# dataexplorations2026/cough_detector

Hardware: AMD Instinct MI355X
Metric: 1s@16kHz clips/sec (featurise+infer) (higher is better)
Workload: dtype bf16x3: split-bf16 MFMA (feature image, activations and BN-folded weights as hi+lo bf16 pairs, 3 v_mfma_f32_32x32x16_bf16 per k-step, f32 accumulate, f32 activations in HBM); featuriser f32

## Files before the change

cough_detector_amd/csrc/featurize.hip:

```cpp
#include <cmath>
#include <cstddef>
#include <cstring>
#include <type_traits>
#include <vector>

#include <hip/hip_bf16.h>

#include <cstdlib>

#include "common.h"
#include "fft256.h"
#include "internal.h"

namespace cough {
namespace {

constexpr int NS = 16000, NFFT = 512, HOP = 160, WIN = 400, NFRAMES = 101, NMEL = 64, NMFCC = 13;
constexpr int PADL = NFFT / 2;
constexpr int NBIN = 128;
constexpr int MAXW = 8;
constexpr int THREADS = 256, WAVES = THREADS / 64;
constexpr int FPW = 4;
constexpr int NGROUP = (NFRAMES + FPW - 1) / FPW;
constexpr int XROW = 17;
constexpr int XFRAME = 16 * XROW;
constexpr int NMF = NMFCC * NFRAMES;
constexpr int FIRST_PLAIN = 2, LAST_PLAIN = 98;

struct FeatTables {
    float win[NFFT];
    float2 tw256[16][16];
    float2 tw512[NBIN];
    int mel_start[NMEL];
    float mel_w[NMEL][MAXW];
    float dct_t[NMFCC + 1][NMEL];
};

constexpr size_t LDS_XCH = size_t(WAVES) * FPW * XFRAME * 4;
constexpr size_t LDS_MEL = size_t(NMEL) * NFRAMES * 4;
constexpr size_t LDS_RED = 16 * 4;
constexpr size_t LDS_TW = size_t(16) * XROW * 8;
constexpr size_t LDS_TOTAL = LDS_XCH + LDS_MEL + LDS_RED + LDS_TW;
static_assert(LDS_TOTAL * 3 <= 160 * 1024, "three workgroups per CU");
static_assert(LDS_XCH >= size_t(2) * NMF * 4, "MFCC / delta buffers alias the transpose scratch");

__device__ __forceinline__ float block_max(float v, float* red, int tid) {
    v = wave_max(v);
    __syncthreads();
    if ((tid & 63) == 0) red[tid >> 6] = v;
    __syncthreads();
    float r = red[0];
#pragma unroll
    for (int w = 1; w < WAVES; ++w) r = fmaxf(r, red[w]);
    return r;
}
__device__ __forceinline__ float block_sum(float v, float* red, int tid) {
    v = wave_sum(v);
    __syncthreads();
    if ((tid & 63) == 0) red[tid >> 6] = v;
    __syncthreads();
    float r = red[0];
#pragma unroll
    for (int w = 1; w < WAVES; ++w) r += red[w];
    return r;
}

#ifdef COUGH_K1_STAMPS
__device__ unsigned long long* g_stamp_buf = nullptr;
#define K1_STAMP(slot)                                                                      \
    do {                                                                                    \
        if (g_stamp_buf && threadIdx.x == 0)                                                \
            g_stamp_buf[(size_t)blockIdx.x * 8 + (slot)] = __builtin_amdgcn_s_memtime();    \
    } while (0)
#else
#define K1_STAMP(slot) do { } while (0)
#endif

#ifdef COUGH_K1_MARKERS
#define K1_MARK(text)                             \
    do {                                          \
        __builtin_amdgcn_sched_barrier(0);        \
        asm volatile("; K1MARK " text);           \
        __builtin_amdgcn_sched_barrier(0);        \
    } while (0)
#else
#define K1_MARK(text) do { } while (0)
#endif

using f32x16 = __attribute__((ext_vector_type(16))) float;
using bf16x8 = __attribute__((ext_vector_type(8))) __bf16;
__device__ __forceinline__ uint16_t f2bf(float f) {
    __hip_bfloat16 b = __float2bfloat16(f);
    return *reinterpret_cast<uint16_t*>(&b);
}
constexpr int ST_P1H = 22, ST_P1W = 25, ST_ROWS = 94, ST_PITCH = 106;
constexpr int ST_PER = ST_P1H * ST_P1W, ST_TILES = (ST_PER + 7) / 8;
constexpr size_t ST_IMG = size_t(ST_ROWS) * ST_PITCH * 2;
static_assert(ST_IMG <= LDS_MEL, "the bf16 feature image aliases the dB buffer");
constexpr size_t ST_X3_OFF = LDS_TOTAL - 2 * ST_IMG;
static_assert(ST_X3_OFF % 16 == 0 && ST_IMG % 4 == 0 && ST_X3_OFF >= size_t(NMF) * 4, "hi / lo images vs the MFCC buffer");

struct FullBank {
    int n_mels, n_mfcc, n_taps;
    int maxw[2];
    int n_frames, n_samples, hop;
    int cph, cph_pad, cw;
    const int *lo, *hi, *off;
    const float* w;
    const float* dct;
};
constexpr size_t full_mel_bytes(int n_mels, int n_frames = NFRAMES) { return (size_t(n_mels) * n_frames * 4 + 15) & ~size_t(15); }
constexpr int FX_ROW = FPW * 16 + 1, FX_WAVE = 16 * FX_ROW, FX_PROW = 260;
static_assert(FPW * FX_PROW <= FX_WAVE && FX_PROW >= NFFT / 2 + 2 && FX_PROW % 2 == 0, "four power rows replace the transposes");
constexpr size_t LDS_XCH_FULL = size_t(WAVES) * FX_WAVE * 4;
constexpr int FULL_MAX_MFCC = int(LDS_XCH_FULL / (size_t(2) * NFRAMES * 4));
constexpr size_t full_lds_bytes(int n_mels, int n_taps, int n_frames = NFRAMES) {
    return LDS_XCH_FULL + full_mel_bytes(n_mels, n_frames) + LDS_RED + LDS_TW + ((size_t(n_taps) * 4 + 15) & ~size_t(15));
}

#ifndef COUGH_GEO_WG_PER_CU
#define COUGH_GEO_WG_PER_CU 2
#endif
template <bool PRE_EMPH, int STEM, bool FULL = false, bool TALL = false, bool PCS = false, bool GEO = false>
__global__ __launch_bounds__(THREADS, GEO ? COUGH_GEO_WG_PER_CU : 3) void featurize_kernel(
    const float* __restrict__ wav, long long wav_stride, float* __restrict__ out, int nfeat,
    const FeatTables* __restrict__ tb, int normalize, float pre_coef, int delta_delta , int pcen, StemFuse stem, FullBank fbk,
    const float* __restrict__ full_dct ,
    float* __restrict__ peak_out ) {
    extern __shared__ __attribute__((aligned(16))) char smem[];
    static_assert(!GEO || (FULL && STEM == 0 && !TALL && !PCS), "run-time geometry: full-band instantiations without a stem");
    const int NF = GEO ? fbk.n_frames : NFRAMES, NGR = GEO ? (fbk.n_frames + FPW - 1) / FPW : NGROUP;
    const int NSMP = GEO ? fbk.n_samples : NS, HP = GEO ? fbk.hop : HOP;
    constexpr int N1A = GEO ? 0 : 1, N1B = GEO ? 16 : 15;
    const int nmel = FULL ? fbk.n_mels : NMEL, nmfcc = FULL ? fbk.n_mfcc : NMFCC, nmf = nmfcc * NF;
    const size_t lds_mel = FULL ? full_mel_bytes(nmel, NF) : LDS_MEL;
    constexpr size_t lds_xch = FULL ? LDS_XCH_FULL : LDS_XCH;
    float* xs = reinterpret_cast<float*>(smem);
    float* melbuf = reinterpret_cast<float*>(smem + lds_xch);
    float* red = reinterpret_cast<float*>(smem + lds_xch + lds_mel);
    float2* twl = reinterpret_cast<float2*>(smem + lds_xch + lds_mel + LDS_RED);
    float* c_w = reinterpret_cast<float*>(smem + lds_xch + lds_mel + LDS_RED + LDS_TW);

    const int tid = threadIdx.x, lane = tid & 63, wave = tid >> 6;
    const long long clip = blockIdx.x;
    const float* x = wav + clip * wav_stride;
    float* o = out + clip * (long long)nfeat * NF;
    const bool wr = out != nullptr;

    K1_STAMP(0);
    K1_STAMP(1);
    K1_MARK("PHASE prologue (window taps, twiddle table, mel taps to registers)");

    const int j = lane & 15, fsub = lane >> 4;
    twl[(tid >> 4) * XROW + (tid & 15)] = tb->tw256[tid >> 4][tid & 15];
    int b_lo[2] = {0, 0}, b_w[2] = {0, 0}, b_band[2] = {0, 0};
    const float* b_taps[2] = {c_w, c_w};
    int fpl1 = FPW;
    if constexpr (FULL) {
        for (int i = tid; i < fbk.n_taps; i += THREADS) c_w[i] = fbk.w[i];
        const int r = nmel - 64;
        fpl1 = r > 32 ? 4 : r > 16 ? 2 : 1;
#pragma unroll
        for (int ps = 0; ps < 2; ++ps) {
            const int mb = ps == 0 ? lane : 64 + (fpl1 == 4 ? lane : fpl1 == 2 ? (lane & 31) : (lane & 15));
            if (mb < nmel) {
                b_band[ps] = mb;
                b_lo[ps] = fbk.lo[mb];
                b_w[ps] = fbk.hi[mb] - b_lo[ps];
                b_taps[ps] = c_w + fbk.off[mb];
            } else {
                b_band[ps] = -1;
            }
        }
    }
    __syncthreads();
    const float2* tw_row = twl + j * XROW;
    const float2 tw_j = tb->tw512[j];
    float mw[MAXW];
#pragma unroll
    for (int q = 0; q < MAXW; ++q) mw[q] = tb->mel_w[lane][q];
    const int mstart = tb->mel_start[lane];

    float* myx = xs + (wave * FPW + fsub) * XFRAME;
    float* myw = xs + wave * FX_WAVE;
    float* fxw = myw + 16 * fsub + j;
    const float* fxr = myw + FX_ROW * j + 16 * fsub;
    float* prow = myw + FX_PROW * fsub;
    float run_max = -INFINITY;
    float peak = 0.f;
    float chk = 0.f;
    auto geo_plain = [&](int g) {
        return HP * (FPW * g) - PADL >= 0 && FPW * g + FPW - 1 < NF && HP * (FPW * g + FPW - 1) - PADL + NFFT <= NSMP;
    };
    [[maybe_unused]] float raw_left = 0.f;
    auto load_group = [&](int g, float2 (&raw)[16]) {
        const int t_raw = FPW * g + fsub;
        const int t = t_raw < NF ? t_raw : NF - 1;
        const int s0 = HP * t - PADL + 2 * j;
        if constexpr (GEO) {
            if (geo_plain(g)) {
#pragma unroll
                for (int n1 = 0; n1 < 16; ++n1) raw[n1] = make_float2(x[s0 + 32 * n1], x[s0 + 32 * n1 + 1]);
                if constexpr (PRE_EMPH) raw_left = s0 - 2 * j > 0 ? x[s0 - 2 * j - 1] : 0.f;
            } else {
#pragma unroll
                for (int n1 = 0; n1 < 16; ++n1) {
                    int i0 = s0 + 32 * n1, i1 = i0 + 1;
                    i0 = i0 < 0 ? -i0 : (i0 >= NSMP ? 2 * (NSMP - 1) - i0 : i0);
                    i1 = i1 < 0 ? -i1 : (i1 >= NSMP ? 2 * (NSMP - 1) - i1 : i1);
                    raw[n1] = make_float2(x[i0], x[i1]);
                }
            }
        } else
        if (FPW * g >= FIRST_PLAIN && FPW * g + FPW - 1 <= LAST_PLAIN) {
            K1_MARK("WEIGHT 0.885 (23 of 26 groups: frames inside the clip)");
#pragma unroll
            for (int n1 = 1; n1 < 15; ++n1) raw[n1] = *reinterpret_cast<const float2*>(x + s0 + 32 * n1);
            K1_MARK("ENDWEIGHT");
        } else {
            K1_MARK("WEIGHT 0.115 (3 of 26 groups: reflected edge frames)");
#pragma unroll
            for (int n1 = 1; n1 < 15; ++n1) {
                int i0 = s0 + 32 * n1, i1 = i0 + 1;
                i0 = i0 < 0 ? -i0 : (i0 >= NS ? 2 * (NS - 1) - i0 : i0);
                i1 = i1 < 0 ? -i1 : (i1 >= NS ? 2 * (NS - 1) - i1 : i1);
                raw[n1] = make_float2(x[i0], x[i1]);
            }
            K1_MARK("ENDWEIGHT");
        }
    };
    float2 raw[16];
    float peak_m = 0.f;
    auto p1_pass = [&](const float ws1, const float ws2) {
        float w_re[16], w_im[16];
        const int jw = 2 * j;
#pragma unroll
        for (int n1 = N1A; n1 < N1B; ++n1) {
            w_re[n1] = tb->win[32 * n1 + jw] * ws1 * ws2;
            w_im[n1] = tb->win[32 * n1 + jw + 1] * ws1 * ws2;
        }
        load_group(wave, raw);

        K1_MARK("LOOP 6.5 P1 four-frame groups per wave");
        for (int g = wave; g < NGR; g += WAVES) {
            K1_MARK("PHASE P1 peak + window multiply + next group's loads");
            const int t_raw = FPW * g + fsub;
// ... 399 lines not shown
    if constexpr (TALL) {
        static_assert(!TALL || STEM == 2, "the 103-row stem: split-bf16 operands");
        constexpr int TL_P1H = 26, TL_HALF = 13, TL_PER = TL_HALF * ST_P1W, TL_ROWS = 58, TL_PLANE = TL_ROWS * ST_PITCH;
        constexpr size_t TL_IMG_OFF = (size_t(2) * NMF * 4 + 15) & ~size_t(15), TL_STASH_OFF = TL_IMG_OFF + size_t(2) * TL_PLANE * 2;
        constexpr int TL_KEEP0 = 2 * 2 * TL_HALF - 3;
        static_assert(TL_STASH_OFF % 16 == 0 && TL_STASH_OFF + size_t(NMEL - TL_KEEP0) * NFRAMES * 4 <= LDS_TOTAL, "103-row stem LDS");
        static_assert(2 * (2 * (TL_HALF - 1) + 1) + 1 + 6 < TL_ROWS && TL_P1H == 2 * TL_HALF, "partial image rows");
        constexpr int NDV = (NMEL * NFRAMES / 2 + THREADS - 1) / THREADS;
        float2 dv[NDV];
#pragma unroll
        for (int it = 0; it < NDV; ++it) {
            const int i2 = tid + it * THREADS;
            dv[it] = i2 < NMEL * NFRAMES / 2 ? reinterpret_cast<const float2*>(melbuf)[i2] : make_float2(0.f, 0.f);
        }
        float* o_mfcc = o + NMEL * NFRAMES;
        float* o_delta = o_mfcc + NMF;
        for (int item = tid; item < NMF; item += THREADS) {
            const int c = item / NFRAMES, t = item - c * NFRAMES;
            const float* row = mf + c * NFRAMES;
            const float d = (row[t < NFRAMES - 1 ? t + 1 : t] - row[t > 0 ? t - 1 : 0]) / 2.0f;
            if (wr) {
                o_mfcc[item] = row[t];
                o_delta[item] = d;
            }
            dl[item] = d;
        }
        __syncthreads();
        auto ddelta = [&](int c, int t) {
            const float* row = dl + c * NFRAMES;
            return (row[t < NFRAMES - 1 ? t + 1 : t] - row[t > 0 ? t - 1 : 0]) / 2.0f;
        };
        if (wr) {
            float* o_dd = o_delta + NMF;
            for (int item = tid; item < NMF; item += THREADS) o_dd[item] = ddelta(item / NFRAMES, item % NFRAMES);
        }
        uint16_t* timg = reinterpret_cast<uint16_t*>(smem + TL_IMG_OFF);
        float* stash = reinterpret_cast<float*>(smem + TL_STASH_OFF);
        auto tput = [&](int idx, float v) {
            const uint16_t hi = f2bf(v);
            timg[idx] = hi;
            timg[TL_PLANE + idx] = f2bf(v - __uint_as_float(uint32_t(hi) << 16));
        };
        auto zero_image = [&]() {
            for (int i = tid; i < 2 * TL_PLANE / 8; i += THREADS) reinterpret_cast<uint4*>(timg)[i] = make_uint4(0, 0, 0, 0);
            for (int i = (2 * TL_PLANE / 8) * 8 + tid; i < 2 * TL_PLANE; i += THREADS) timg[i] = 0;
            __syncthreads();
        };
        zero_image();
        if constexpr (PCS) {
            const int m = tid >> 2, t0 = (tid & 3) * 26;
#pragma unroll
            for (int k = 0; k < 26; ++k) {
                if (t0 + k < NFRAMES) {
                    if (m + 3 < TL_ROWS - 1) tput((m + 3) * ST_PITCH + t0 + k + 3, pcv[k]);
                    if (m >= TL_KEEP0) stash[(m - TL_KEEP0) * NFRAMES + t0 + k] = pcv[k];
                }
            }
        } else {
            {
#pragma unroll
                for (int it = 0; it < NDV; ++it) {
                    const int e = 2 * (tid + it * THREADS);
                    if (e < NMEL * NFRAMES) {
                        const int m0 = e / NFRAMES, t0 = e - m0 * NFRAMES;
                        const int m1 = t0 + 1 < NFRAMES ? m0 : m0 + 1, t1 = t0 + 1 < NFRAMES ? t0 + 1 : 0;
                        const float v0 = fminf(fmaxf((dv[it].x + 80.0f) * 0.0125f, 0.f), 1.f);
                        const float v1 = fminf(fmaxf((dv[it].y + 80.0f) * 0.0125f, 0.f), 1.f);
                        if (m0 + 3 < TL_ROWS - 1) tput((m0 + 3) * ST_PITCH + t0 + 3, v0);
                        if (m1 + 3 < TL_ROWS - 1) tput((m1 + 3) * ST_PITCH + t1 + 3, v1);
                        if (m0 >= TL_KEEP0) stash[(m0 - TL_KEEP0) * NFRAMES + t0] = v0;
                        if (m1 >= TL_KEEP0) stash[(m1 - TL_KEEP0) * NFRAMES + t1] = v1;
                    }
                }
            }
        }
        const int sr = lane & 31, sh = lane >> 5;
        bf16x8 bw[2][4];
#pragma unroll
        for (int pl = 0; pl < 2; ++pl)
#pragma unroll
            for (int st = 0; st < 4; ++st)
                bw[pl][st] = *reinterpret_cast<const bf16x8*>(stem.wfrag + pl * 2048 + ((st * 2 + sh) * 32 + sr) * 8);
        const float bn = stem.bias[sr];
        const int q = sr >> 2, dy = (sr >> 1) & 1, dx = sr & 1;
        float* oa = reinterpret_cast<float*>(stem.a1) + clip * (long long)(TL_P1H * ST_P1W) * 32;
#pragma unroll 1
        for (int half = 0; half < 2; ++half) {
            if (half == 1) {
                zero_image();
                for (int i = tid; i < (NMEL - TL_KEEP0) * NFRAMES; i += THREADS) {
                    const int m = i / NFRAMES, t = i - m * NFRAMES;
                    tput(m * ST_PITCH + t + 3, stash[i]);
                }
                for (int item = tid; item < NMF; item += THREADS) {
                    const int c = item / NFRAMES, t = item - c * NFRAMES;
                    tput((NMEL - TL_KEEP0 + c) * ST_PITCH + t + 3, mf[item]);
                    tput((NMEL - TL_KEEP0 + NMFCC + c) * ST_PITCH + t + 3, dl[item]);
                    tput((NMEL - TL_KEEP0 + 2 * NMFCC + c) * ST_PITCH + t + 3, ddelta(c, t));
                }
            }
            __syncthreads();
            auto tl_base = [&](int tile) -> const uint32_t* {
                int P = tile * 8 + q;
                if (P >= TL_PER) P = TL_PER - 1;
                const int ph = P / ST_P1W, pw = P - ph * ST_P1W;
                return reinterpret_cast<const uint32_t*>(timg + (2 * (2 * ph + dy) + sh) * ST_PITCH + 2 * (2 * pw + dx));
            };
            auto tl_load = [&](const uint32_t* base, bf16x8 (&fa)[2][4]) {
#pragma unroll
                for (int pl = 0; pl < 2; ++pl)
#pragma unroll
                    for (int st = 0; st < 4; ++st) {
                        const uint32_t* pp = base + pl * (TL_PLANE / 2) + st * ST_PITCH;
                        union { uint32_t u[4]; bf16x8 v; } tv;
                        tv.u[0] = pp[0]; tv.u[1] = pp[1]; tv.u[2] = pp[2]; tv.u[3] = pp[3];
                        fa[pl][st] = tv.v;
                    }
            };
            auto tl_mma = [&](const bf16x8 (&fa)[2][4], f32x16& c) {
#pragma unroll
                for (int st = 0; st < 4; ++st) {
                    c = __builtin_amdgcn_mfma_f32_32x32x16_bf16(fa[0][st], bw[0][st], c, 0, 0, 0);
                    c = __builtin_amdgcn_mfma_f32_32x32x16_bf16(fa[1][st], bw[0][st], c, 0, 0, 0);
                    c = __builtin_amdgcn_mfma_f32_32x32x16_bf16(fa[0][st], bw[1][st], c, 0, 0, 0);
                }
            };
            auto tl_store = [&](int tile, const f32x16& acc2) {
#pragma unroll
                for (int g = 0; g < 4; ++g) {
                    const int Po = tile * 8 + 2 * g + sh;
                    float v = fmaxf(fmaxf(acc2[4 * g], acc2[4 * g + 1]), fmaxf(acc2[4 * g + 2], acc2[4 * g + 3])) + bn;
                    v = fmaxf(v, 0.f);
                    if (Po < TL_PER) oa[(half * TL_PER + Po) * 32 + sr] = v;
                }
            };
            constexpr int TL_TILES = (TL_PER + 7) / 8;
            for (int ta = wave; ta < TL_TILES; ta += 2 * WAVES) {
                const int tb = ta + WAVES;
                const bool two = tb < TL_TILES;
                bf16x8 fa[2][4], fb[2][4];
                tl_load(tl_base(ta), fa);
                tl_load(tl_base(two ? tb : ta), fb);
                f32x16 ca = {0}, cb = {0};
                tl_mma(fa, ca);
                tl_mma(fb, cb);
                tl_store(ta, ca);
                if (two) tl_store(tb, cb);
            }
            __syncthreads();
        }
        return;
    }
    if constexpr (STEM != 0) {
        float2 dv[(NMEL * NFRAMES / 2 + THREADS - 1) / THREADS];
#pragma unroll
        for (int it = 0; it < (NMEL * NFRAMES / 2 + THREADS - 1) / THREADS; ++it) {
            const int i2 = tid + it * THREADS;
            dv[it] = i2 < NMEL * NFRAMES / 2 ? reinterpret_cast<const float2*>(melbuf)[i2] : make_float2(0.f, 0.f);
        }
        __syncthreads();
        constexpr int NIMG = STEM == 2 ? 2 : 1;
        for (int i = tid; i < NIMG * ST_ROWS * ST_PITCH / 8; i += THREADS) reinterpret_cast<uint4*>(img)[i] = make_uint4(0, 0, 0, 0);
        for (int i = (NIMG * ST_ROWS * ST_PITCH / 8) * 8 + tid; i < NIMG * ST_ROWS * ST_PITCH; i += THREADS) img[i] = 0;
        __syncthreads();
        if constexpr (PCS) {
            const int m = tid >> 2, t0 = (tid & 3) * 26;
#pragma unroll
            for (int k = 0; k < 26; ++k)
                if (t0 + k < NFRAMES) put((m + 3) * ST_PITCH + t0 + k + 3, pcv[k]);
        } else {
#pragma unroll
            for (int it = 0; it < (NMEL * NFRAMES / 2 + THREADS - 1) / THREADS; ++it) {
                const int e = 2 * (tid + it * THREADS);
                if (e < NMEL * NFRAMES) {
                    const int m0 = e / NFRAMES, t0 = e - m0 * NFRAMES;
                    const int m1 = t0 + 1 < NFRAMES ? m0 : m0 + 1, t1 = t0 + 1 < NFRAMES ? t0 + 1 : 0;
                    put((m0 + 3) * ST_PITCH + t0 + 3, fminf(fmaxf((dv[it].x + 80.0f) * 0.0125f, 0.f), 1.f));
                    put((m1 + 3) * ST_PITCH + t1 + 3, fminf(fmaxf((dv[it].y + 80.0f) * 0.0125f, 0.f), 1.f));
                }
            }
        }
    }
    float* o_mfcc = o + nmel * NF;
    float* o_delta = o_mfcc + nmf;
    for (int item = tid; item < nmf; item += THREADS) {
        const int c = item / NF, t = item - c * NF;
        const float* row = mf + c * NF;
        const float d = (row[t < NF - 1 ? t + 1 : t] - row[t > 0 ? t - 1 : 0]) / 2.0f;
        if (wr) {
            o_mfcc[item] = row[t];
            o_delta[item] = d;
        }
        if (delta_delta == 1) dl[item] = d;
        if constexpr (STEM != 0) {
            put((NMEL + c + 3) * ST_PITCH + t + 3, row[t]);
            put((NMEL + NMFCC + c + 3) * ST_PITCH + t + 3, d);
        }
    }
    K1_STAMP(6);
    if (delta_delta == 1 && wr) {
        __syncthreads();
        float* o_dd = o_delta + nmf;
        for (int item = tid; item < nmf; item += THREADS) {
            const int c = item / NF, t = item - c * NF;
            const float* row = dl + c * NF;
            o_dd[item] = (row[t < NF - 1 ? t + 1 : t] - row[t > 0 ? t - 1 : 0]) / 2.0f;
        }
    }
    if constexpr (STEM != 0) {
        __syncthreads();
        K1_MARK("PHASE K2 stem MFMA + pool + store");
        constexpr int NP = STEM == 2 ? 2 : 1;
        const int sr = lane & 31, sh = lane >> 5;
        bf16x8 bw[NP][4];
#pragma unroll
        for (int pl = 0; pl < NP; ++pl)
#pragma unroll
            for (int st = 0; st < 4; ++st)
                bw[pl][st] = *reinterpret_cast<const bf16x8*>(stem.wfrag + pl * 2048 + ((st * 2 + sh) * 32 + sr) * 8);
        const float bn = stem.bias[sr];
        const int q = sr >> 2, dy = (sr >> 1) & 1, dx = sr & 1;
        using out_t = std::conditional_t<STEM == 2, float, uint16_t>;
        out_t* oa = reinterpret_cast<out_t*>(stem.a1) + clip * (long long)ST_PER * 32;
        auto frag_base = [&](int tile) -> const uint32_t* {
            int P = tile * 8 + q;
            if (P >= ST_PER) P = ST_PER - 1;
            const int ph = P / ST_P1W, pw = P - ph * ST_P1W;
            return reinterpret_cast<const uint32_t*>(img + (2 * (2 * ph + dy) + sh) * ST_PITCH + 2 * (2 * pw + dx));
        };
        auto load_frags = [&](const uint32_t* base, bf16x8 (&a)[NP][4]) {
#pragma unroll
            for (int pl = 0; pl < NP; ++pl)
#pragma unroll
                for (int st = 0; st < 4; ++st) {
                    const uint32_t* p = base + pl * (ST_ROWS * ST_PITCH / 2) + st * ST_PITCH;
                    union { uint32_t u[4]; bf16x8 v; } t;
                    t.u[0] = p[0]; t.u[1] = p[1]; t.u[2] = p[2]; t.u[3] = p[3];
                    a[pl][st] = t.v;
                }
        };
        auto mma = [&](const bf16x8 (&a)[NP][4], f32x16& c) {
#pragma unroll
            for (int st = 0; st < 4; ++st) {
                c = __builtin_amdgcn_mfma_f32_32x32x16_bf16(a[0][st], bw[0][st], c, 0, 0, 0);
                if constexpr (STEM == 2) {
                    c = __builtin_amdgcn_mfma_f32_32x32x16_bf16(a[1][st], bw[0][st], c, 0, 0, 0);
                    c = __builtin_amdgcn_mfma_f32_32x32x16_bf16(a[0][st], bw[1][st], c, 0, 0, 0);
                }
            }
        };
        auto epilogue = [&](int tile, const f32x16& acc2, bool guard) {
#pragma unroll
            for (int g = 0; g < 4; ++g) {
                const int Po = tile * 8 + 2 * g + sh;
                float v = fmaxf(fmaxf(acc2[4 * g], acc2[4 * g + 1]), fmaxf(acc2[4 * g + 2], acc2[4 * g + 3])) + bn;
                v = fmaxf(v, 0.f);
                if (!guard || Po < ST_PER) {
                    if constexpr (STEM == 2) oa[Po * 32 + sr] = v;
                    else oa[Po * 32 + sr] = f2bf(v);
                }
            }
        };
        static_assert(ST_TILES == 17 * WAVES + 1, "stem tile split");
        for (int it = 0; it < 16; it += 2) {
            const int ta = wave + WAVES * it, tbb = ta + WAVES;
            bf16x8 fa[NP][4], fb[NP][4];
            load_frags(frag_base(ta), fa);
            load_frags(frag_base(tbb), fb);
            f32x16 ca = {0}, cb = {0};
            mma(fa, ca);
            mma(fb, cb);
            epilogue(ta, ca, false);
            epilogue(tbb, cb, false);
        }
        {
            const int ta = wave + WAVES * 16;
            const bool last = wave == 0;
            bf16x8 fa[NP][4], fb[NP][4];
            load_frags(frag_base(ta), fa);
            load_frags(frag_base(last ? ST_TILES - 1 : ta), fb);
            f32x16 ca = {0}, cb = {0};
            mma(fa, ca);
            mma(fb, cb);
            epilogue(ta, ca, false);
            if (last) epilogue(ST_TILES - 1, cb, true);
        }
        K1_STAMP(7);
    }
}

}
}

struct cough_featurizer {
    cough_feat_config cfg;
    cough::FeatTables* d_tables;
    float* d_win_full;
    int nfeat;
    int nbase;
    cough::ContrastCfg contrast;
    int n_cus;
    int path;
    char* d_full;
    cough::FullBank full;
    cough::GenFeat* gen;
};

namespace cough {
namespace {
bool geo_basic(const cough_feat_config& c) {
    return c.n_fft == NFFT && c.win_length >= 1 && c.win_length <= NFFT && c.hop_length >= 1 && c.n_mels >= 2 && c.n_mels <= 128 &&
           (!c.use_mfcc || (c.n_mfcc >= 1 && c.n_mfcc <= c.n_mels));
}
bool geo_fits(const cough_feat_config& c, int n_taps, int n) {
    if (n <= NFFT / 2) return false;
    const long long T = n / c.hop_length + 1;
    const bool covered = c.hop_length <= NFFT / 2 || (c.hop_length <= NFFT && (T - 1) * c.hop_length + NFFT / 2 >= n);
    return covered && T <= 1024 && (!c.use_pcen || T <= 208) && (!c.use_mfcc || size_t(c.n_mfcc) * T * 4 <= LDS_XCH_FULL) &&
           full_lds_bytes(c.n_mels, n_taps, int(T)) <= 80 * 1024;
}

using K1Fn = decltype(&featurize_kernel<false, 0>);
struct K1Entry {
    bool pe;
    int stem;
    bool full, tall, pcs, geo;
    K1Fn fn;
};
#define K1(PE, STEM, FULL, TALL, PCS, GEO) {PE, STEM, FULL, TALL, PCS, GEO, featurize_kernel<PE, STEM, FULL, TALL, PCS, GEO>}
#define K1_X3(FULL, PCS) K1(false, 2, FULL, false, PCS, false), K1(false, 2, FULL, true, PCS, false), \
                        K1(true, 2, FULL, false, PCS, false), K1(true, 2, FULL, true, PCS, false)
const K1Entry K1_TABLE[] = {
    K1(false, 0, true, false, false, false), K1(true, 0, true, false, false, false),
    K1_X3(true, false), K1_X3(true, true),
    K1(false, 0, true, false, false, true), K1(true, 0, true, false, false, true),
    K1_X3(false, false), K1_X3(false, true),
    K1(false, 1, false, false, false, false),
    K1(true, 0, false, false, false, false), K1(false, 0, false, false, false, false),
};
#undef K1_X3
#undef K1
static_assert(sizeof(K1_TABLE) / sizeof(K1_TABLE[0]) == 23, "one entry per instantiation");
K1Fn k1_kernel(bool pe, int stem, bool full, bool tall, bool pcs, bool geo) {
    for (const K1Entry& k : K1_TABLE)
        if (k.pe == pe && k.stem == stem && k.full == full && k.tall == tall && k.pcs == pcs && k.geo == geo) return k.fn;
    return nullptr;
}

bool shipped_stft(const cough_feat_config& c) {
    return c.n_fft == NFFT && c.hop_length == HOP && c.win_length == WIN && c.segment_samples == NS;
}
struct Band {
    int first, last;
};
std::vector<Band> scan_bands(const cough_feat_config& c, const float* mel_fb) {
    std::vector<Band> bands(c.n_fft == NFFT && c.n_mels > 0 ? c.n_mels : 0, Band{-1, -1});
    for (int k = 0; !bands.empty() && k <= NFFT / 2; ++k)
        for (int m = 0; m < c.n_mels; ++m)
            if (mel_fb[k * c.n_mels + m] != 0.f) {
                if (bands[m].first < 0) bands[m].first = k;
                bands[m].last = k;
            }
    return bands;
}

int segment_path(const cough_feat_config& c, const std::vector<Band>& bands, int n_taps) {
    bool stft = shipped_stft(c);
    for (int i = 0; c.use_spectral_contrast && i < c.n_contrast_bands; ++i)
        stft = stft && c.contrast_edges[i + 1] - c.contrast_edges[i] <= 128;
    bool regs = stft && c.n_mels == NMEL && c.n_mfcc == NMFCC;
    for (const Band& b : bands) regs = regs && (b.first < 0 || (b.last < NBIN && b.last - b.first < MAXW));
    if (regs) return COUGH_PATH_TUNED;
    const bool basic = geo_basic(c);
    if (stft && basic && c.n_mels % 2 == 0 && (!c.use_mfcc || c.n_mfcc <= FULL_MAX_MFCC) && (!c.use_pcen || c.n_mels == NMEL) &&
        full_lds_bytes(c.n_mels, n_taps, NFRAMES) <= 80 * 1024)
        return COUGH_PATH_TUNED_FULLBAND;
    return basic && geo_fits(c, n_taps, c.segment_samples) ? COUGH_PATH_TUNED_GEOMETRY : COUGH_PATH_GENERIC;
}

FeatTables shipped_tables(const cough_feat_config& c, const float* window, const float* mel_fb, const float* dct,
                          const std::vector<Band>& bands, int path) {
    FeatTables t{};
    const double PI = 3.14159265358979323846;
    if (shipped_stft(c) || geo_basic(c)) {
        const int left = (NFFT - c.win_length) / 2;
        for (int n = 0; n < c.win_length; ++n) t.win[left + n] = window[n];
        for (int jj = 0; jj < 16; ++jj)
            for (int k1 = 0; k1 < 16; ++k1) {
                const double a = -2.0 * PI * double(jj * k1) / 256.0;
                t.tw256[jj][k1] = make_float2(float(std::cos(a)), float(std::sin(a)));
            }
        for (int k = 0; k < NBIN; ++k) {
            const double a = -2.0 * PI * double(k) / 512.0;
            t.tw512[k] = make_float2(float(std::cos(a)), float(std::sin(a)));
        }
    }
    if (path == COUGH_PATH_TUNED) {
        for (int m = 0; m < NMEL; ++m) {
            int first = bands[m].first < 0 ? 0 : bands[m].first;
            if (first > NBIN - MAXW) first = NBIN - MAXW;
            t.mel_start[m] = first;
            for (int q = 0; q < MAXW; ++q) t.mel_w[m][q] = 0.25f * mel_fb[(first + q) * NMEL + m];
        }
        for (int c2 = 0; c2 < NMFCC; ++c2)
            for (int m = 0; m < NMEL; ++m) t.dct_t[c2][m] = dct[m * NMFCC + c2];
    }
    return t;
}

struct HostBank {
    FullBank fb{};
    std::vector<int> lo, hi, off;
    std::vector<float> taps, dct;
};
HostBank csr_bank(const cough_feat_config& c, const float* mel_fb, const float* dct, const std::vector<Band>& bands) {
    HostBank h;
    FullBank& fb = h.fb;
    const int nm = c.n_mels, nc = c.use_mfcc ? c.n_mfcc : 1;
    fb.n_mels = nm;
    fb.n_mfcc = nc;
    for (int m = 0; m < nm; ++m) {
        const int first = bands[m].first < 0 ? 0 : bands[m].first, last = bands[m].first < 0 ? -1 : bands[m].last;
        const int lo2 = first & ~1, hi2 = last >= first ? (last + 2) & ~1 : lo2;
        h.lo.push_back(lo2);
        h.hi.push_back(hi2);
        h.off.push_back(hi2 > lo2 ? int(h.taps.size()) : 0);
        for (int k = lo2; k < hi2; ++k) h.taps.push_back(k >= first && k <= last ? 0.25f * mel_fb[k * nm + m] : 0.f);
        const int w = (hi2 - lo2 + 3) / 4 * 4;
        if (w > fb.maxw[m >> 6]) fb.maxw[m >> 6] = w;
    }
    if (h.taps.size() < 2) h.taps.assign(2, 0.f);
    fb.n_taps = int(h.taps.size());
    fb.cph = (nc + 1) / 2;
    const int n_chunks = (fb.cph + 6) / 7;
    fb.cw = (fb.cph + n_chunks - 1) / n_chunks;
    if (fb.cw < 4) fb.cw = 4;
    fb.cph_pad = (fb.cph + fb.cw - 1) / fb.cw * fb.cw;
    const int chunks_per_half = fb.cph_pad / fb.cw;
// ... 216 lines not shown
```

Measured before the change: 6.365 million.

## Build stem feature image with packed bf16 row writes and incremental tile offsets

Replaces the zero-fill-then-scatter construction of the bf16 hi/lo feature image with per-wave whole-row writes of packed bf16 pairs, padding zeros included. This removes one barrier and the separate clear pass, and folds the MFCC/delta image writes into the same row writer. The MFCC output loop is skipped when nothing needs writing. In the stem MFMA loop, per-tile fragment base addresses are advanced incrementally instead of recomputed, and the tail tile no longer issues redundant MFMAs on waves other than 0. The risk is that the layout assumptions behind the hard-coded row and lane mapping are wrong, which would corrupt the image.

```diff
diff --git a/cough_detector_amd/csrc/featurize.hip b/cough_detector_amd/csrc/featurize.hip
--- a/cough_detector_amd/csrc/featurize.hip
+++ b/cough_detector_amd/csrc/featurize.hip
@@ -92,6 +92,13 @@
 __device__ __forceinline__ uint16_t f2bf(float f) {
     __hip_bfloat16 b = __float2bfloat16(f);
     return *reinterpret_cast<uint16_t*>(&b);
+}
+__device__ __forceinline__ uint32_t pk_bf16(float a, float b) {
+    typedef __bf16 bf16x2_t __attribute__((ext_vector_type(2)));
+    typedef float f32x2_t __attribute__((ext_vector_type(2)));
+    const f32x2_t v = {a, b};
+    const bf16x2_t p = __builtin_convertvector(v, bf16x2_t);
+    return __builtin_bit_cast(uint32_t, p);
 }
 constexpr int ST_P1H = 22, ST_P1W = 25, ST_ROWS = 94, ST_PITCH = 106;
 constexpr int ST_PER = ST_P1H * ST_P1W, ST_TILES = (ST_PER + 7) / 8;
@@ -797,49 +804,75 @@
         return;
     }
     if constexpr (STEM != 0) {
-        float2 dv[(NMEL * NFRAMES / 2 + THREADS - 1) / THREADS];
-#pragma unroll
-        for (int it = 0; it < (NMEL * NFRAMES / 2 + THREADS - 1) / THREADS; ++it) {
-            const int i2 = tid + it * THREADS;
-            dv[it] = i2 < NMEL * NFRAMES / 2 ? reinterpret_cast<const float2*>(melbuf)[i2] : make_float2(0.f, 0.f);
+        constexpr int RDW = ST_PITCH / 2;
+        constexpr int NOTHER = ST_ROWS - NMEL;
+        static_assert(ST_PITCH % 2 == 0 && RDW <= 64 && 2 * RDW - 3 >= NFRAMES && NMEL % WAVES == 0, "image dword layout");
+        static_assert(ST_ROWS == 3 + NMEL + 2 * NMFCC + 1, "image rows");
+        const int k = min(lane, RDW - 1), t0 = 2 * k - 3, t1 = t0 + 1;
+        const bool ok0 = t0 >= 0 && t0 < NFRAMES, ok1 = t1 >= 0 && t1 < NFRAMES;
+        const int c0 = min(max(t0, 0), NFRAMES - 1), c1 = min(max(t1, 0), NFRAMES - 1);
+        const int fw = (wave + 1) & 3;
+        uint32_t* img32 = reinterpret_cast<uint32_t*>(img);
+        auto put2 = [&](int row, float v0, float v1) {
+            const uint32_t hi = pk_bf16(v0, v1);
+            img32[row * RDW + k] = hi;
+            if constexpr (STEM == 2)
+                img32[ST_ROWS * RDW + row * RDW + k] = pk_bf16(v0 - __uint_as_float(hi << 16), v1 - __uint_as_float(hi & 0xffff0000u));
+        };
+        float2 sv[NMEL / WAVES];
+#pragma unroll
+        for (int i = 0; i < NMEL / WAVES; ++i) {
+            const float* mrow = melbuf + (4 * i + fw) * NFRAMES;
+            sv[i] = make_float2(mrow[c0], mrow[c1]);
         }
         __syncthreads();
-        constexpr int NIMG = STEM == 2 ? 2 : 1;
-        for (int i = tid; i < NIMG * ST_ROWS * ST_PITCH / 8; i += THREADS) reinterpret_cast<uint4*>(img)[i] = make_uint4(0, 0, 0, 0);
-        for (int i = (NIMG * ST_ROWS * ST_PITCH / 8) * 8 + tid; i < NIMG * ST_ROWS * ST_PITCH; i += THREADS) img[i] = 0;
-        __syncthreads();
+#pragma unroll
+        for (int i = 0; i < NMEL / WAVES; ++i) {
+            const float v0 = !PCS && ok0 ? fminf(fmaxf((sv[i].x + 80.0f) * 0.0125f, 0.f), 1.f) : 0.f;
+            const float v1 = !PCS && ok1 ? fminf(fmaxf((sv[i].y + 80.0f) * 0.0125f, 0.f), 1.f) : 0.f;
+            put2(4 * i + fw + 3, v0, v1);
+        }
+#pragma unroll
+        for (int j = 0; j < (NOTHER + WAVES - 1) / WAVES; ++j) {
+            const int x = wave + WAVES * j;
+            if (x < NOTHER) {
+                float v0 = 0.f, v1 = 0.f;
+                if (x >= 3 && x < 3 + 2 * NMFCC) {
+                    const int c = x < 3 + NMFCC ? x - 3 : x - 3 - NMFCC;
+                    const float* row = mf + c * NFRAMES;
+                    if (x < 3 + NMFCC) {
+                        v0 = row[c0];
+                        v1 = row[c1];
+                    } else {
+                        v0 = (row[min(c0 + 1, NFRAMES - 1)] - row[max(c0 - 1, 0)]) / 2.0f;
+                        v1 = (row[min(c1 + 1, NFRAMES - 1)] - row[max(c1 - 1, 0)]) / 2.0f;
+                    }
+                    v0 = ok0 ? v0 : 0.f;
+                    v1 = ok1 ? v1 : 0.f;
+                }
+                put2(x < 3 ? x : x + NMEL, v0, v1);
+            }
+        }
         if constexpr (PCS) {
-            const int m = tid >> 2, t0 = (tid & 3) * 26;
-#pragma unroll
-            for (int k = 0; k < 26; ++k)
-                if (t0 + k < NFRAMES) put((m + 3) * ST_PITCH + t0 + k + 3, pcv[k]);
-        } else {
-#pragma unroll
-            for (int it = 0; it < (NMEL * NFRAMES / 2 + THREADS - 1) / THREADS; ++it) {
-                const int e = 2 * (tid + it * THREADS);
-                if (e < NMEL * NFRAMES) {
-                    const int m0 = e / NFRAMES, t0 = e - m0 * NFRAMES;
-                    const int m1 = t0 + 1 < NFRAMES ? m0 : m0 + 1, t1 = t0 + 1 < NFRAMES ? t0 + 1 : 0;
-                    put((m0 + 3) * ST_PITCH + t0 + 3, fminf(fmaxf((dv[it].x + 80.0f) * 0.0125f, 0.f), 1.f));
-                    put((m1 + 3) * ST_PITCH + t1 + 3, fminf(fmaxf((dv[it].y + 80.0f) * 0.0125f, 0.f), 1.f));
-                }
-            }
+            __syncthreads();
+            const int m = tid >> 2, tq = (tid & 3) * 26;
+#pragma unroll
+            for (int kk = 0; kk < 26; ++kk)
+                if (tq + kk < NFRAMES) put((m + 3) * ST_PITCH + tq + kk + 3, pcv[kk]);
         }
     }
     float* o_mfcc = o + nmel * NF;
     float* o_delta = o_mfcc + nmf;
-    for (int item = tid; item < nmf; item += THREADS) {
-        const int c = item / NF, t = item - c * NF;
-        const float* row = mf + c * NF;
-        const float d = (row[t < NF - 1 ? t + 1 : t] - row[t > 0 ? t - 1 : 0]) / 2.0f;
-        if (wr) {
-            o_mfcc[item] = row[t];
-            o_delta[item] = d;
-        }
-        if (delta_delta == 1) dl[item] = d;
-        if constexpr (STEM != 0) {
-            put((NMEL + c + 3) * ST_PITCH + t + 3, row[t]);
-            put((NMEL + NMFCC + c + 3) * ST_PITCH + t + 3, d);
+    if (wr || delta_delta == 1) {
+        for (int item = tid; item < nmf; item += THREADS) {
+            const int c = item / NF, t = item - c * NF;
+            const float* row = mf + c * NF;
+            const float d = (row[t < NF - 1 ? t + 1 : t] - row[t > 0 ? t - 1 : 0]) / 2.0f;
+            if (wr) {
+                o_mfcc[item] = row[t];
+                o_delta[item] = d;
+            }
+            if (delta_delta == 1) dl[item] = d;
         }
     }
     K1_STAMP(6);
@@ -907,11 +940,30 @@
             }
         };
         static_assert(ST_TILES == 17 * WAVES + 1, "stem tile split");
+        constexpr int STEP = 8 * WAVES, DPH = STEP / ST_P1W, DPW = STEP - DPH * ST_P1W;
+        static_assert(DPH == 1 && DPW == 7, "tile stride");
+        int pw, fo;
+        {
+            const int P = wave * 8 + q, ph = P / ST_P1W;
+            pw = P - ph * ST_P1W;
+            fo = (4 * ph + 2 * dy + sh) * ST_PITCH + 4 * pw + 2 * dx;
+        }
+        auto advance = [&]() {
+            pw += DPW;
+            fo += 4 * DPH * ST_PITCH + 4 * DPW;
+            if (pw >= ST_P1W) {
+                pw -= ST_P1W;
+                fo += 4 * ST_PITCH - 4 * ST_P1W;
+            }
+        };
+        auto at = [&](int off) { return reinterpret_cast<const uint32_t*>(img + off); };
         for (int it = 0; it < 16; it += 2) {
             const int ta = wave + WAVES * it, tbb = ta + WAVES;
             bf16x8 fa[NP][4], fb[NP][4];
-            load_frags(frag_base(ta), fa);
-            load_frags(frag_base(tbb), fb);
+            load_frags(at(fo), fa);
+            advance();
+            load_frags(at(fo), fb);
+            advance();
             f32x16 ca = {0}, cb = {0};
             mma(fa, ca);
             mma(fb, cb);
@@ -920,15 +972,21 @@
         }
         {
             const int ta = wave + WAVES * 16;
-            const bool last = wave == 0;
-            bf16x8 fa[NP][4], fb[NP][4];
-            load_frags(frag_base(ta), fa);
-            load_frags(frag_base(last ? ST_TILES - 1 : ta), fb);
-            f32x16 ca = {0}, cb = {0};
-            mma(fa, ca);
-            mma(fb, cb);
-            epilogue(ta, ca, false);
-            if (last) epilogue(ST_TILES - 1, cb, true);
+            bf16x8 fa[NP][4];
+            load_frags(at(fo), fa);
+            f32x16 ca = {0};
+            if (wave == 0) {
+                bf16x8 fb[NP][4];
+                load_frags(frag_base(ST_TILES - 1), fb);
+                f32x16 cb = {0};
+                mma(fa, ca);
+                mma(fb, cb);
+                epilogue(ta, ca, false);
+                epilogue(ST_TILES - 1, cb, true);
+            } else {
+                mma(fa, ca);
+                epilogue(ta, ca, false);
+            }
         }
         K1_STAMP(7);
     }
```

Result: faster. 6.433 million, median of 6 (+1.1%).
